# FAKEBOB-adversarial-attack/FAKEBOB

Hardware: AMD Instinct MI355X
Metric: NES iterations/sec (and scored-utts/sec) at samples_per_draw=50, 3 s@16 kHz (higher is better)
Workload: dtype f32 (GMM: two-term f16 split on MFMA, f32 accumulate, f32-equivalent; f32 MFCC; f64 NES)

## Files before the change

fakebob_amd/csrc/gmm_wide_kernel.hip:

```cpp
#include <float.h>
#include <cstdlib>
#include <type_traits>

#include "fb_kernels.h"
#include "gmm_split.h"

__device__ __forceinline__ void fb_glds16(const void *gsrc, unsigned lds_dst) {
  unsigned keep;
  asm volatile("s_mov_b32 %0, m0\n\ts_mov_b32 m0, %2\n\ts_nop 0\n\tglobal_load_lds_dwordx4 %1, off\n\ts_mov_b32 m0, %0"
               : "=&s"(keep) : "v"(gsrc), "s"(lds_dst) : "memory");
}
template <int N>
__device__ __forceinline__ void fb_glds16_run(const void *gsrc, unsigned lds_dst) {
  unsigned keep;
#define FB_GLDS_HEAD "s_mov_b32 %0, m0\n\ts_mov_b32 m0, %2\n\ts_nop 0\n\tglobal_load_lds_dwordx4 %1, off\n\t"
#define FB_GLDS_AT(o) "global_load_lds_dwordx4 %1, off offset:" #o "\n\t"
#define FB_GLDS_TAIL "s_mov_b32 m0, %0"
  if constexpr (N == 1)
    asm volatile(FB_GLDS_HEAD FB_GLDS_TAIL : "=&s"(keep) : "v"(gsrc), "s"(lds_dst) : "memory");
  else if constexpr (N == 2)
    asm volatile(FB_GLDS_HEAD FB_GLDS_AT(1024) FB_GLDS_TAIL : "=&s"(keep) : "v"(gsrc), "s"(lds_dst) : "memory");
  else if constexpr (N == 3)
    asm volatile(FB_GLDS_HEAD FB_GLDS_AT(1024) FB_GLDS_AT(2048) FB_GLDS_TAIL : "=&s"(keep) : "v"(gsrc), "s"(lds_dst) : "memory");
  else
    asm volatile(FB_GLDS_HEAD FB_GLDS_AT(1024) FB_GLDS_AT(2048) FB_GLDS_AT(3072) FB_GLDS_TAIL
                 : "=&s"(keep) : "v"(gsrc), "s"(lds_dst) : "memory");
#undef FB_GLDS_HEAD
#undef FB_GLDS_AT
#undef FB_GLDS_TAIL
}
template <int NITEMS, int NPIECE>
__device__ __forceinline__ void fb_fxw_fetch(const u32x4 *__restrict__ group_lane, unsigned lds_dst, int wv) {
  constexpr int TOT = NITEMS * NPIECE, PW = (TOT + 3) / 4;
  const u32x4 *src = group_lane + (size_t)wv * (PW * 64);
  const unsigned dst = lds_dst + (unsigned)wv * (PW * 1024);
// ... 10 lines not shown
__device__ __forceinline__ float fb_v_fma(float a, float b, float c) {
  float d;
  asm volatile("v_fma_f32 %0, %1, %2, %3" : "=v"(d) : "v"(a), "v"(b), "v"(c));
  return d;
}
__device__ __forceinline__ float fb_v_exp(float a) {
  float d;
  asm volatile("v_exp_f32 %0, %1" : "=v"(d) : "v"(a));
  return d;
}
__device__ __forceinline__ float fb_v_add(float a, float b) {
  float d;
  asm volatile("v_add_f32 %0, %1, %2" : "=v"(d) : "v"(a), "v"(b));
  return d;
}

#ifdef FB_FXW_COUNT
__device__ unsigned long long g_fxw_counts[4];
extern "C" int fb_debug_fxw_counts(unsigned long long *out) {
  if (hipMemcpyFromSymbol(out, HIP_SYMBOL(g_fxw_counts), sizeof(g_fxw_counts)) != hipSuccess) return -1;
  unsigned long long z[4] = {0, 0, 0, 0};
  return hipMemcpyToSymbol(HIP_SYMBOL(g_fxw_counts), z, sizeof(z)) == hipSuccess ? 0 : -1;
}
#define FXW_COUNT(i) do { if ((threadIdx.x & 63) == 0) atomicAdd(&g_fxw_counts[i], 1ull); } while (0)
#else
#define FXW_COUNT(i) do { } while (0)
#endif
#ifdef FB_FXW_STAMP
__device__ unsigned long long g_fxw_stamps[16];
extern "C" int fb_debug_fxw_stamps(unsigned long long *out) {
  return hipMemcpyFromSymbol(out, HIP_SYMBOL(g_fxw_stamps), sizeof(g_fxw_stamps)) == hipSuccess ? 0 : -1;
}
#define FXW_STAMP(i) do { if (blockIdx.x == 8 && threadIdx.x == 0) g_fxw_stamps[i] = wall_clock64(); } while (0)
#else
#define FXW_STAMP(i) do { } while (0)
#endif
#define FB_FXW_ROFF 64.0f
#define FB_FXW_SMAX 1.2676506002282294e30f
struct FbFxwUpd { float so0, so1, sn0, sn1; };

__device__ __forceinline__ void fb_fxw_slow_update(const f32x16 &p, float up, float rt, float mo, float so,
                                                   float *__restrict__ pm, float *__restrict__ ps, float &rn, bool need) {
  float tm = -3.0e38f;
#pragma unroll
  for (int r = 0; r < 16; ++r) tm = fmaxf(tm, __fmul_rn(p[r], up));
  const float mo_e = so > 0.0f ? mo : -INFINITY;
  const float mn = fmaxf(mo_e, __fadd_rn(rt, rintf(tm)));
  const float off = __fsub_rn(mn, rt);
  float a0 = __fmul_rn(so, __builtin_amdgcn_exp2f(__fsub_rn(mo_e, mn))), a1 = 0.0f;
#pragma unroll
  for (int r = 0; r < 16; r += 2) {
    a0 = __fadd_rn(a0, __builtin_amdgcn_exp2f(__fmaf_rn(p[r], up, -off)));
    a1 = __fadd_rn(a1, __builtin_amdgcn_exp2f(__fmaf_rn(p[r + 1], up, -off)));
  }
  if (need) {
    *pm = mn;
    *ps = __fadd_rn(a0, a1);
    rn = fmaxf(rn, mn);
  }
}

template <int NK, int NP, bool UPD, bool ZI = false, bool DEFERRED = false>
__device__ __forceinline__ void fb_fxw_step(const u32x4 *__restrict__ cur4, const u32x4 *__restrict__ nxt4, const bool pf0,
                                            int lane, u32x4 &z1, u32x4 &z2, const u32x4 (&b1)[2][NK],
                                            const u32x4 (&b2)[2][NK], const f32x16 &init0, const f32x16 &init1,
                                            f32x16 &out0, f32x16 &out1, const f32x16 &p0, const f32x16 &p1,
                                            float *__restrict__ ps, const float wd0, const float wd1, FbFxwUpd &u,
                                            const u32x4 *__restrict__ dsrc, unsigned ddst, const int dq0, const int dn) {
  constexpr int KP = 2 * NP, NG = KP * NK;
  constexpr int NS = 20;
  static_assert(NP >= 1 && NP <= 3 && NG >= 10, "slice layout");
  f32x16 x0, x1;
  if constexpr (ZI) {
#pragma unroll
    for (int r = 0; r < 16; ++r) { x0[r] = 0.0f; x1[r] = 0.0f; }
  } else {
    x0 = init0;
    x1 = init1;
  }
  constexpr int PD = NP == 1 ? 2 : 1;
  u32x4 s1[PD + 1], s2[PD + 1];
  float se0 = 0.f, se1 = 0.f, sd0 = 0.f, sd1 = 0.f;
  float ea0 = 0.f, ea1 = 0.f, eb0 = 0.f, eb1 = 0.f;
#pragma unroll
  for (int g = 0; g < NG; ++g) {
    const int c = g / KP, kk = g % KP;
    const int k = NP == 3 ? kk : (NP == 2 ? (kk < 2 ? kk : kk + 2) : kk + 4);
    if (kk == 0) {
#pragma unroll
      for (int cn = (c == 0 ? 1 : c + PD); cn <= c + PD && cn < NK; ++cn) {
        s1[cn % (PD + 1)] = cur4[(0 * NK + cn) * 64 + lane];
        if (NP >= 2) s2[cn % (PD + 1)] = cur4[(1 * NK + cn) * 64 + lane];
      }
    }
    const u32x4 &a1 = c == 0 ? z1 : s1[c % (PD + 1)], &a2 = c == 0 ? z2 : s2[c % (PD + 1)];
    if (k == 0) FB_FX_MFMA(a2, b1[0][c], x0);
    else if (k == 1) FB_FX_MFMA(a2, b1[1][c], x1);
    else if (k == 2) FB_FX_MFMA(a1, b2[0][c], x0);
    else if (k == 3) FB_FX_MFMA(a1, b2[1][c], x1);
    else if (k == 4) FB_FX_MFMA(a1, b1[0][c], x0);
    else FB_FX_MFMA(a1, b1[1][c], x1);
    if (pf0 && g == KP + 1) {
      z1 = nxt4[(0 * NK + 0) * 64 + lane];
      z2 = nxt4[(1 * NK + 0) * 64 + lane];
    }
    if (kk == (KP > 3 ? 3 : KP - 1) && c < dn) fb_glds16(dsrc + (dq0 + c) * 64, ddst + (unsigned)(dq0 + c) * 1024u);
    if constexpr (UPD) {
      const int m0 = (g * 4 * NS) / NG, m1 = ((g + 1) * 4 * NS) / NG;
#pragma unroll
      for (int mm = m0; mm < m1; ++mm) {
        const int sl = mm >> 2, part = mm & 3;
        const int r = sl - 1;
        const int ra = sl - 3;
        if (part == 0) {
          if (ra == 0) se0 = ea0;
          else if (ra == 1) sd0 = ea0;
          else if (ra >= 2 && ra <= 15 && !(ra & 1)) se0 = fb_v_add(se0, ea0);
          else if (ra >= 2 && ra <= 15) sd0 = fb_v_add(sd0, ea0);
        } else if (part == 1) {
          if (ra == 0) se1 = ea1;
          else if (ra == 1) sd1 = ea1;
          else if (ra >= 2 && ra <= 15 && !(ra & 1)) se1 = fb_v_add(se1, ea1);
          else if (ra >= 2 && ra <= 15) sd1 = fb_v_add(sd1, ea1);
          ea0 = eb0; ea1 = eb1;
        } else if (part == 2) {
          if (sl == 0) { u.so0 = ps[0]; u.so1 = ps[256]; }
          if (r >= 0 && r <= 15) eb0 = fb_v_exp(p0[r]);
        } else {
          if (r >= 0 && r <= 15) eb1 = fb_v_exp(p1[r]);
          if (sl == NS - 1) {
            u.sn0 = DEFERRED ? fb_v_fma(fb_v_add(se0, sd0), wd0, u.so0) : fb_v_add(fb_v_add(se0, sd0), u.so0);
            u.sn1 = DEFERRED ? fb_v_fma(fb_v_add(se1, sd1), wd1, u.so1) : fb_v_add(fb_v_add(se1, sd1), u.so1);
            ps[0] = u.sn0; ps[256] = u.sn1;
          }
        }
      }
    }
    __builtin_amdgcn_sched_barrier(0);
  }
  asm volatile("" : "+v"(x0), "+v"(x1));
  out0 = x0;
  out1 = x1;
}


typedef int i32x8 __attribute__((ext_vector_type(8)));
template <int NK, bool UPD>
__device__ __forceinline__ void fb_fxw_step6(const u32x4 *__restrict__ cur4, const u32x4 *__restrict__ nxt4, const bool pf0,
                                             int lane, u32x4 &z1, const u32x4 (&b1)[2][NK], const i32x8 (&fq)[2][3],
                                             const int (&fsc)[2][3], const f32x16 &init0, const f32x16 &init1,
                                             f32x16 &out0, f32x16 &out1, const f32x16 &p0, const f32x16 &p1,
                                             float *__restrict__ ps, FbFxwUpd &u, const u32x4 *__restrict__ dsrc, unsigned ddst,
                                             const int dq0, const int dn) {
  static_assert(NK == 5, "F6 item layout");
  constexpr int NM = 2 * NK, NG = NM + 8;
  constexpr int NS = 20, PD = 2;
  f32x16 x0 = init0, x1 = init1;
  u32x4 s1[PD + 1];
  i32x8 pa[4];
  int psc = 0, psh[4] = {0, 0, 0, 0};
  float se0 = 0.f, se1 = 0.f, sd0 = 0.f, sd1 = 0.f;
  float ea0 = 0.f, ea1 = 0.f, eb0 = 0.f, eb1 = 0.f;
  const unsigned char *ib = reinterpret_cast<const unsigned char *>(cur4);
#pragma unroll
  for (int g = 0; g < NG; ++g) {
    if (g < NM) {
      const int c = g / 2, kk = g % 2;
      if (kk == 0) {
#pragma unroll
        for (int cn = (c == 0 ? 1 : c + PD); cn <= c + PD && cn < NK; ++cn) s1[cn % (PD + 1)] = cur4[cn * 64 + lane];
        if (c == 0) {
          const u32x4 lo = *reinterpret_cast<const u32x4 *>(ib + 5120 + lane * 16);
          const uint2 hi = *reinterpret_cast<const uint2 *>(ib + 6144 + lane * 8);
          pa[0] = i32x8{(int)lo[0], (int)lo[1], (int)lo[2], (int)lo[3], (int)hi.x, (int)hi.y, 0, 0};
          psc = *reinterpret_cast<const int *>(ib + 9984 + lane * 4);
        } else if (c == 1) {
          const u32x4 lo = *reinterpret_cast<const u32x4 *>(ib + 8192 + lane * 16);
          pa[1] = i32x8{(int)lo[0], (int)lo[1], (int)lo[2], (int)lo[3], 0, 0, 0, 0};
        } else if (c == 2) {
          const u32x4 lo = *reinterpret_cast<const u32x4 *>(ib + 6656 + lane * 16);
          const uint2 hi = *reinterpret_cast<const uint2 *>(ib + 7680 + lane * 8);
          pa[2] = i32x8{(int)lo[0], (int)lo[1], (int)lo[2], (int)lo[3], (int)hi.x, (int)hi.y, 0, 0};
        } else if (c == 3) {
          const u32x4 lo = *reinterpret_cast<const u32x4 *>(ib + 9216 + (lane & 31) * 16);
          const uint2 hi = *reinterpret_cast<const uint2 *>(ib + 9728 + (lane & 31) * 8);
          pa[3] = i32x8{(int)lo[0], (int)lo[1], (int)lo[2], (int)lo[3], (int)hi.x, (int)hi.y, 0, 0};
        } else {
          psh[0] = psc; psh[1] = psc >> 16; psh[2] = psc >> 8; psh[3] = psc >> 24;
        }
      }
      const u32x4 &a1 = c == 0 ? z1 : s1[c % (PD + 1)];
      if (kk == 0) FB_FX_MFMA(a1, b1[0][c], x0);
      else FB_FX_MFMA(a1, b1[1][c], x1);
      if (pf0 && g == 3) z1 = nxt4[lane];
      if (kk == 1 && c < dn) fb_glds16(dsrc + (dq0 + c) * 64, ddst + (unsigned)(dq0 + c) * 1024u);
    } else {
      const int blk = (g - NM) / 2, hf = (g - NM) % 2;
      const int fb = blk == 0 || blk == 1 ? 0 : blk - 1;
      const int sa = psh[blk];
      if (blk == 1) {
        if (hf == 0) x0 = __builtin_amdgcn_mfma_scale_f32_32x32x64_f8f6f4(pa[1], fq[0][fb], x0, 4, 2, 0, sa, 0, fsc[0][fb]);
        else x1 = __builtin_amdgcn_mfma_scale_f32_32x32x64_f8f6f4(pa[1], fq[1][fb], x1, 4, 2, 0, sa, 0, fsc[1][fb]);
      } else {
        if (hf == 0) x0 = __builtin_amdgcn_mfma_scale_f32_32x32x64_f8f6f4(pa[blk], fq[0][fb], x0, 2, 2, 0, sa, 0, fsc[0][fb]);
        else x1 = __builtin_amdgcn_mfma_scale_f32_32x32x64_f8f6f4(pa[blk], fq[1][fb], x1, 2, 2, 0, sa, 0, fsc[1][fb]);
      }
    }
    if constexpr (UPD) {
      const int m0 = (g * 4 * NS) / NG, m1 = ((g + 1) * 4 * NS) / NG;
#pragma unroll
      for (int mm = m0; mm < m1; ++mm) {
        const int sl = mm >> 2, part = mm & 3;
        const int r = sl - 1, ra = sl - 3;
        if (part == 0) {
          if (ra == 0) se0 = ea0;
          else if (ra == 1) sd0 = ea0;
          else if (ra >= 2 && ra <= 15 && !(ra & 1)) se0 = fb_v_add(se0, ea0);
          else if (ra >= 2 && ra <= 15) sd0 = fb_v_add(sd0, ea0);
        } else if (part == 1) {
          if (ra == 0) se1 = ea1;
          else if (ra == 1) sd1 = ea1;
          else if (ra >= 2 && ra <= 15 && !(ra & 1)) se1 = fb_v_add(se1, ea1);
          else if (ra >= 2 && ra <= 15) sd1 = fb_v_add(sd1, ea1);
          ea0 = eb0; ea1 = eb1;
        } else if (part == 2) {
          if (sl == 0) { u.so0 = ps[0]; u.so1 = ps[256]; }
          if (r >= 0 && r <= 15) eb0 = fb_v_exp(p0[r]);
        } else {
          if (r >= 0 && r <= 15) eb1 = fb_v_exp(p1[r]);
          if (sl == NS - 1) {
            u.sn0 = fb_v_add(fb_v_add(se0, sd0), u.so0);
            u.sn1 = fb_v_add(fb_v_add(se1, sd1), u.so1);
            ps[0] = u.sn0; ps[256] = u.sn1;
          }
        }
      }
    }
    __builtin_amdgcn_sched_barrier(0);
  }
  asm volatile("" : "+v"(x0), "+v"(x1));
  out0 = x0;
  out1 = x1;
}

template <int NK, int M>
__global__ __launch_bounds__(256, 1) void k_gmm_fx2w(FbGmmDev g, const float *__restrict__ feats,
                                                     const int *__restrict__ n_rows_ptr, int n_chunks,
                                                     int rows_cap, float *__restrict__ part_m,
                                                     float *__restrict__ part_s, int xcd_map) {
  if (g.stop && *g.stop) return;
  extern __shared__ __attribute__((aligned(16))) float lds[];
  constexpr int IMG4 = 2 * NK * 64;
  constexpr int NI = M + 1;
  constexpr int GA = (NI + 1) / 2, GB = NI - GA;
  FXW_STAMP(0);
  const int n_rows = *n_rows_ptr;
  int strip_i, gchunk;
  if (xcd_map) {
    const int lin = blockIdx.x, per = 8 / xcd_map;
    const int xcd = lin & 7, idx = lin >> 3;
    gchunk = xcd / per;
    strip_i = idx * per + (xcd % per);
  } else {
    strip_i = blockIdx.x;
    gchunk = blockIdx.y;
  }
  const int n_sub = g.fxw_sub > 1 ? g.fxw_sub : 1, grid_chunks = n_chunks / n_sub;
  const int strip0 = strip_i * 256;
  if (strip0 >= n_rows) return;
  const int tid = threadIdx.x, lane = tid & 63, w = tid >> 6;
  const int h = lane >> 5, j = lane & 31;
  constexpr int PAD4 = 192;
  constexpr int SLOTB4 = GA * IMG4 + PAD4;
  const u32x4 *slot0 = reinterpret_cast<const u32x4 *>(lds);
  float *st_m = lds + (NI * IMG4 + 2 * PAD4) * 4;
  float *st_s = st_m + M * 512;
// ... 236 lines not shown
  const int wv = __builtin_amdgcn_readfirstlane(w);
  const unsigned ring_lds = (unsigned)(unsigned long long)(__attribute__((address_space(3))) void *)lds;
  auto item4 = [&](int jj) { return jj < GA ? jj * IMG4 : SLOTB4 + (jj - GA) * IMG4; };
  const unsigned guard = slow ? 0u : __float_as_uint(FB_FXW_SMAX) + 1u;
  auto settle = [&](const f32x16 &p0, const f32x16 &p1, float *pm, float *ps, const float (&rt)[2], const FbFxwUpd &u) {
    const unsigned worst = max(__float_as_uint(u.sn0), __float_as_uint(u.sn1));
    FXW_COUNT(0);
#ifdef FB_FXW_COUNT
    {
      const float th0 = __builtin_amdgcn_logf(u.so0) - 25.0f, th1 = __builtin_amdgcn_logf(u.so1) - 25.0f;
      int n = 0;
#pragma unroll
      for (int r = 0; r < 16; ++r)
        if (__builtin_amdgcn_ballot_w64(!(p0[r] < th0) || !(p1[r] < th1)) == 0ull) ++n;
      if ((threadIdx.x & 63) == 0) atomicAdd(&g_fxw_counts[3], (unsigned long long)n);
    }
#endif
    if (__builtin_expect(__builtin_amdgcn_ballot_w64(worst >= guard) != 0ull, 0)) {
      FXW_COUNT(1);
      fb_fxw_slow_update(p0, up[0], rt[0], pm[0], u.so0, pm, ps, rn[0], __float_as_uint(u.sn0) >= guard);
      fb_fxw_slow_update(p1, up[1], rt[1], pm[256], u.so1, pm + 256, ps + 256, rn[1], __float_as_uint(u.sn1) >= guard);
    }
  };
  auto update = [&](const f32x16 &v0, const f32x16 &v1, int model) {
    float *pm = st_m + (2 * model) * 256 + tid, *ps = st_s + (2 * model) * 256 + tid;
    fb_fxw_slow_update(v0, up[0], rc[0], pm[0], ps[0], pm, ps, rn[0], true);
    fb_fxw_slow_update(v1, up[1], rc[1], pm[256], ps[256], pm + 256, ps + 256, rn[1], true);
  };
  auto publish = [&]() {
    asm volatile("s_waitcnt vmcnt(0)" ::: "memory");
    __syncthreads();
  };

  f32x16 hq[2], acc[2][2], zero;
#pragma unroll
  for (int r = 0; r < 16; ++r) {
    hq[0][r] = 0.f; hq[1][r] = 0.f; zero[r] = 0.f;
    acc[0][0][r] = -1.0e30f; acc[0][1][r] = -1.0e30f; acc[1][0][r] = -1.0e30f; acc[1][1][r] = -1.0e30f;
  }
  FbFxwUpd uu;
  float wd[2] = {1.0f, 1.0f};
  FXW_STAMP(3);
  fb_fxw_fetch<GA, NPIECE>(gimg + (size_t)tile_of(0) * NI * IMG4 + lane, ring_lds, wv);
  publish();
  FXW_STAMP(4);
  u32x4 z1, z2;
  constexpr int PW_A = (GA * NPIECE + 3) / 4, PW_B = (GB * NPIECE + 3) / 4;
  auto tile = [&](auto pc, const int t) __attribute__((always_inline)) {
    constexpr int P = decltype(pc)::value;
    rp[0] = rc[0]; rp[1] = rc[1];
    if (__builtin_expect(__builtin_amdgcn_ballot_w64(rn[0] > rc[0] || rn[1] > rc[1] || wd[0] != 1.0f || wd[1] != 1.0f) != 0ull, 0)) {
      FXW_COUNT(2);
#pragma unroll
      for (int hf = 0; hf < 2; ++hf) {
        rn[hf] = fminf(fmaxf(rn[hf], __shfl_xor(rn[hf], 32, 64)), 4.0e6f);
        rc[hf] = slow ? 0.0f : rn[hf];
        set_ref(hf, rc[hf]);
        wd[hf] = __builtin_amdgcn_exp2f(rp[hf] - rc[hf]);
        if (!slow) {
#pragma unroll
          for (int m = 0; m < M; ++m) {
            float *pm = st_m + (2 * m + hf) * 256 + tid, *ps = st_s + (2 * m + hf) * 256 + tid;
            *ps = *ps * __builtin_amdgcn_exp2f(*pm - rc[hf]);
            *pm = rc[hf];
          }
        }
      }
    }
    const u32x4 *srcB = gimg + ((size_t)tile_of(t) * NI + GA) * IMG4 + (size_t)wv * (PW_B * 64) + lane;
    const u32x4 *srcA = gimg + (size_t)tile_of(t + 1) * NI * IMG4 + (size_t)wv * (PW_A * 64) + lane;
    const unsigned dstB = ring_lds + SLOTB4 * 16 + (unsigned)wv * (PW_B * 1024), dstA = ring_lds + (unsigned)wv * (PW_A * 1024);
#pragma clang loop unroll(full)
    for (int jj = 0; jj < NI; ++jj) {
      const bool first_of_group = (jj == 0 || jj == GA);
      const u32x4 *cur4 = slot0 + item4(jj);
      if (first_of_group) {
        z1 = cur4[(0 * NK + 0) * 64 + lane];
        z2 = cur4[(1 * NK + 0) * 64 + lane];
      }
      const int gs = jj < GA ? jj : jj - GA;
      const int pw = jj < GA ? PW_B : PW_A, dq0 = 5 * gs;
      int dn = dq0 < pw ? (pw - dq0 < 5 ? pw - dq0 : 5) : 0;
      const u32x4 *dsrc = jj < GA ? srcB : srcA;
      const unsigned ddst = jj < GA ? dstB : dstA;
      if (first_of_group) {
#pragma unroll
        for (int q = 0; q < dn; ++q) fb_glds16(dsrc + q * 64, ddst + (unsigned)q * 1024u);
        dn = 0;
      }
      const bool pf0 = (jj + 1 < NI && jj + 1 != GA);
      const u32x4 *nxt4 = slot0 + item4(jj + 1 < NI ? jj + 1 : 0);
      constexpr bool DEFER = M >= 3;
      if (jj == 0) {
        if constexpr (DEFER) {
          float *pm = st_m + (2 * (M - 2)) * 256 + tid, *ps = st_s + (2 * (M - 2)) * 256 + tid;
          fb_fxw_step<NK, 3, true, true, true>(cur4, nxt4, pf0, lane, z1, z2, bq1, bq2, zero, zero, hq[0], hq[1], acc[(M - 2) & 1][0], acc[(M - 2) & 1][1], ps, wd[0], wd[1], uu, dsrc, ddst, dq0, dn);
          settle(acc[(M - 2) & 1][0], acc[(M - 2) & 1][1], pm, ps, rp, uu);
        } else {
          fb_fxw_step<NK, 3, false, true>(cur4, nxt4, pf0, lane, z1, z2, bq1, bq2, zero, zero, hq[0], hq[1], zero, zero, st_s, 1.f, 1.f, uu, dsrc, ddst, dq0, dn);
        }
      } else if (jj == 1) {
        float *pm = st_m + (2 * (M - 1)) * 256 + tid, *ps = st_s + (2 * (M - 1)) * 256 + tid;
        fb_fxw_step<NK, 3, true, false, true>(cur4, nxt4, pf0, lane, z1, z2, bx1, bx2, hq[0], hq[1], hq[0], hq[1], acc[(M - 1) & 1][0], acc[(M - 1) & 1][1], ps, wd[0], wd[1], uu, dsrc, ddst, dq0, dn);
        settle(acc[(M - 1) & 1][0], acc[(M - 1) & 1][1], pm, ps, rp, uu);
      } else if (jj == 2) {
        float *pm = st_m + tid, *ps = st_s + tid;
        if constexpr (P == 6)
          fb_fxw_step6<NK, true>(cur4, nxt4, pf0, lane, z1, bx1, fq, fsc, hq[0], hq[1], acc[1][0], acc[1][1], hq[0], hq[1], ps, uu, dsrc, ddst, dq0, dn);
        else
          fb_fxw_step<NK, P, true>(cur4, nxt4, pf0, lane, z1, z2, bx1, bx2, hq[0], hq[1], acc[1][0], acc[1][1], hq[0], hq[1], ps, 1.f, 1.f, uu,
                                   dsrc, ddst, dq0, dn);
        settle(hq[0], hq[1], pm, ps, rc, uu);
      } else if (DEFER && jj == NI - 1) {
        if constexpr (P == 6)
          fb_fxw_step6<NK, false>(cur4, nxt4, pf0, lane, z1, bx1, fq, fsc, hq[0], hq[1], acc[(jj - 1) & 1][0], acc[(jj - 1) & 1][1],
                                  zero, zero, st_s, uu, dsrc, ddst, dq0, dn);
        else
          fb_fxw_step<NK, P, false>(cur4, nxt4, pf0, lane, z1, z2, bx1, bx2, hq[0], hq[1], acc[(jj - 1) & 1][0], acc[(jj - 1) & 1][1],
                                    zero, zero, st_s, 1.f, 1.f, uu, dsrc, ddst, dq0, dn);
      } else {
        float *pm = st_m + (2 * (jj - 2)) * 256 + tid, *ps = st_s + (2 * (jj - 2)) * 256 + tid;
        if constexpr (P == 6)
          fb_fxw_step6<NK, true>(cur4, nxt4, pf0, lane, z1, bx1, fq, fsc, hq[0], hq[1], acc[(jj - 1) & 1][0], acc[(jj - 1) & 1][1],
                                 acc[(jj - 2) & 1][0], acc[(jj - 2) & 1][1], ps, uu, dsrc, ddst, dq0, dn);
        else
          fb_fxw_step<NK, P, true>(cur4, nxt4, pf0, lane, z1, z2, bx1, bx2, hq[0], hq[1], acc[(jj - 1) & 1][0], acc[(jj - 1) & 1][1],
                                   acc[(jj - 2) & 1][0], acc[(jj - 2) & 1][1], ps, 1.f, 1.f, uu, dsrc, ddst, dq0, dn);
        settle(acc[(jj - 2) & 1][0], acc[(jj - 2) & 1][1], pm, ps, rc, uu);
      }
      if (jj == GA - 1 || jj == NI - 1) publish();
    }
  };
  {
    int t = 0;
    for (; t < n_p3; ++t) tile(std::integral_constant<int, 3>{}, t);
    for (; t < n_p36; ++t) tile(std::integral_constant<int, 6>{}, t);
    for (; t < n_p32; ++t) tile(std::integral_constant<int, 2>{}, t);
    for (; t < n_t; ++t) tile(std::integral_constant<int, 1>{}, t);
  }
  FXW_STAMP(5);
  asm volatile("s_waitcnt vmcnt(0)" ::: "memory");
  auto tail_update = [&](const f32x16 &v0, const f32x16 &v1, int model) {
    if (slow) { update(v0, v1, model); return; }
    float *pm = st_m + (2 * model) * 256 + tid, *ps = st_s + (2 * model) * 256 + tid;
    FbFxwUpd u;
    u.so0 = ps[0]; u.so1 = ps[256];
    float e0 = __builtin_amdgcn_exp2f(v0[0]), d0 = __builtin_amdgcn_exp2f(v0[1]);
    float e1 = __builtin_amdgcn_exp2f(v1[0]), d1 = __builtin_amdgcn_exp2f(v1[1]);
#pragma unroll
    for (int r = 2; r < 16; r += 2) {
      e0 = __fadd_rn(e0, __builtin_amdgcn_exp2f(v0[r])); d0 = __fadd_rn(d0, __builtin_amdgcn_exp2f(v0[r + 1]));
      e1 = __fadd_rn(e1, __builtin_amdgcn_exp2f(v1[r])); d1 = __fadd_rn(d1, __builtin_amdgcn_exp2f(v1[r + 1]));
    }
    u.sn0 = __fadd_rn(__fadd_rn(e0, d0), u.so0);
    u.sn1 = __fadd_rn(__fadd_rn(e1, d1), u.so1);
    ps[0] = u.sn0; ps[256] = u.sn1;
    settle(v0, v1, pm, ps, rc, u);
  };
  if constexpr (M >= 3) tail_update(acc[(M - 2) & 1][0], acc[(M - 2) & 1][1], M - 2);
  tail_update(acc[(M - 1) & 1][0], acc[(M - 1) & 1][1], M - 1);
  FXW_STAMP(6);

#pragma unroll
  for (int m = 0; m < M; ++m)
#pragma unroll
    for (int hf = 0; hf < 2; ++hf) {
      const float ms = st_m[(2 * m + hf) * 256 + tid], s0 = st_s[(2 * m + hf) * 256 + tid];
      const float ln2f = 0.693147182464599609375f;
      const float mm = __fmul_rn(ms, ln2f);
      const float dd = __fmaf_rn(ms, -1.9046542999e-9f, __fmaf_rn(ms, ln2f, -mm));
      const float ss = __fmaf_rn(s0, __fmaf_rn(__fmul_rn(0.5f, dd), dd, dd), s0);
      const float m2 = __shfl_xor(mm, 32, 64), s2 = __shfl_xor(ss, 32, 64);
      const float mx = fmaxf(mm, m2);
      const float sx = ss * __expf(mm - mx) + s2 * __expf(m2 - mx);
      if (h == 0 && rows[hf] < n_rows) {
        const int mg = m == 0 ? 0 : g.pass_first + m - 1;
        const size_t o = ((size_t)chunk_i * g.M + mg) * rows_cap + rows[hf];
        part_m[o] = mx;
        part_s[o] = sx;
      }
    }
  }
  FXW_STAMP(7);
}


template <int NK, bool PICK>
__global__ __launch_bounds__(256, 1) void k_gsel_w(FbGmmDev g, const float *__restrict__ feats, const int *__restrict__ n_rows_ptr,
                                                   int tiles_per_chunk, int n_chunks, float *__restrict__ gmax,
                                                   const float *__restrict__ tau, float *__restrict__ gval,
                                                   unsigned char *__restrict__ gid, int *__restrict__ gcnt, int xcd_map,
                                                   int tiles_a) {
  if (g.stop && *g.stop) return;
// ... 35 lines not shown
    fb_fx_frame_load<NK>(g, feats, rows[hf], n_rows, h, ft[hf]);
  }
#pragma unroll
  for (int hf = 0; hf < 2; ++hf) {
    (void)fb_fx_frame_make<NK, true>(g, feats, ft[hf], rows[hf], n_rows, h, bx1[hf], bx2[hf], bq1[hf], bq2[hf]);
#pragma unroll
    for (int c = 0; c < NK; ++c) asm volatile("" : "+a"(bx2[hf][c]), "+a"(bq1[hf][c]), "+a"(bq2[hf][c]));
    __builtin_amdgcn_sched_barrier(0);
  }
  FXW_STAMP(9);
  float tauv[2] = {FLT_MAX, FLT_MAX};
  float4 *gb[2] = {nullptr, nullptr};
  if constexpr (PICK) {
#pragma unroll
    for (int hf = 0; hf < 2; ++hf) {
      if (rows[hf] < n_rows) tauv[hf] = tau[rows[hf]];
      gb[hf] = reinterpret_cast<float4 *>(gval) + ((size_t)(rows[hf] < n_rows ? rows[hf] : 0) * n_chunks + chunk_i) * capc * 4;
    }
    s_cnt[tid] = 0;
  }
  const int tile0 = chunk_i * tiles_per_chunk;
  const int n_tiles_run = PICK ? tiles_per_chunk : tiles_a;
  const int n_grp = n_tiles_run / TS;
  const u32x4 *gimg = g.images_fx + (size_t)tile0 * 2 * IMG4;
  const int wv = __builtin_amdgcn_readfirstlane(w);
  const unsigned ring_lds = (unsigned)(unsigned long long)(__attribute__((address_space(3))) void *)lds;
  auto publish = [&]() {
    asm volatile("s_waitcnt vmcnt(0)" ::: "memory");
    __syncthreads();
  };
  f32x16 hq[2][2], zero;
#pragma unroll
  for (int r = 0; r < 16; ++r) { hq[0][0][r] = 0.f; hq[0][1][r] = 0.f; hq[1][0][r] = 0.f; hq[1][1][r] = 0.f; zero[r] = 0.f; }
  FbFxwUpd uu;
  FXW_STAMP(10);
  fb_fxw_fetch<NIG, NPIECE>(gimg + lane, ring_lds, wv);
  publish();
  FXW_STAMP(11);
  u32x4 z1, z2;
  auto epilogue = [&](const int tl, const int par) {
#pragma unroll
    for (int hf = 0; hf < 2; ++hf) {
      const f32x16 &v = hq[par][hf];
      float m = fmaxf(fmaxf(v[0], v[1]), v[2]);
#pragma unroll
      for (int r = 3; r < 15; r += 2) m = fmaxf(fmaxf(m, v[r]), v[r + 1]);
      m = fmaxf(m, v[15]);
      if constexpr (!PICK) {
        s_mx[((w * 16 + (tl & 15)) * 2 + hf) * 64 + lane] = m;
      } else {
        if (m >= tauv[hf]) {
          const int rl = w * 64 + hf * 32 + j;
          const int k = atomicAdd(&s_cnt[rl], 1);
          float4 *dst = gb[hf] + (size_t)k * 4;
          dst[0] = make_float4(v[0], v[1], v[2], v[3]);
          dst[1] = make_float4(v[4], v[5], v[6], v[7]);
          dst[2] = make_float4(v[8], v[9], v[10], v[11]);
          dst[3] = make_float4(v[12], v[13], v[14], v[15]);
          s_gid[rl * capc + k] = (unsigned char)(2 * tl + h);
        }
      }
    }
    if constexpr (!PICK) {
      if ((tl & 15) == 15 || tl == tiles_a - 1) {
        const int nt = (tl & 15) + 1, per_row = 2 * nt, NGr = 2 * n_chunks * tiles_a, pos0 = 2 * (chunk_i * tiles_a + (tl & ~15));
        __builtin_amdgcn_fence(__ATOMIC_RELEASE, "wavefront");
        __builtin_amdgcn_wave_barrier();
// ... 7 lines not shown
        __builtin_amdgcn_wave_barrier();
        __builtin_amdgcn_fence(__ATOMIC_ACQUIRE, "wavefront");
      }
    }
  };
  for (int gp = 0; gp < n_grp; gp += 2) {
    const u32x4 *srcB = gimg + (size_t)min(gp + 1, n_grp - 1) * SLOT4 + (size_t)wv * (PW * 64) + lane;
    const u32x4 *srcA = gimg + (size_t)min(gp + 2, n_grp - 1) * SLOT4 + (size_t)wv * (PW * 64) + lane;
    const unsigned dstB = ring_lds + SLOT4 * 16 + (unsigned)wv * (PW * 1024), dstA = ring_lds + (unsigned)wv * (PW * 1024);
#pragma clang loop unroll(full)
    for (int jj = 0; jj < 2 * NIG; ++jj) {
      const bool in_b = jj >= NIG;
      const int gs = jj % NIG;
      const u32x4 *cur4 = slot0 + (in_b ? SLOT4 : 0) + gs * IMG4;
      const u32x4 *nxt4 = slot0 + (in_b ? SLOT4 : 0) + (gs + 1 < NIG ? gs + 1 : 0) * IMG4;
      const bool pf0 = gs + 1 < NIG;
      if (gs == 0) {
        z1 = cur4[(0 * NK + 0) * 64 + lane];
        z2 = cur4[(1 * NK + 0) * 64 + lane];
      }
      const u32x4 *dsrc = in_b ? srcA : srcB;
      const unsigned ddst = in_b ? dstA : dstB;
      const int dq0 = 5 * gs;
      int dn = dq0 < PW ? (PW - dq0 < 5 ? PW - dq0 : 5) : 0;
      if (gs == 0) {
#pragma unroll
        for (int q = 0; q < dn; ++q) fb_glds16(dsrc + q * 64, ddst + (unsigned)q * 1024u);
        dn = 0;
      }
      constexpr int dummy = 0; (void)dummy;
      const int par = (jj >> 1) & 1;
      const int tl = gp * TS + (jj >> 1);
      if (!(jj & 1)) {
        fb_fxw_step<NK, 3, false, true>(cur4, nxt4, pf0, lane, z1, z2, bq1, bq2, zero, zero, hq[par][0], hq[par][1], zero, zero, lds, 1.f, 1.f,
                                        uu, dsrc, ddst, dq0, dn);
        if (tl > 0) epilogue(tl - 1, par ^ 1);
      } else {
        fb_fxw_step<NK, 3, false, false>(cur4, nxt4, pf0, lane, z1, z2, bx1, bx2, hq[par][0], hq[par][1], hq[par][0], hq[par][1], zero, zero, lds,
                                         1.f, 1.f, uu, dsrc, ddst, dq0, dn);
      }
      if (gs == NIG - 1) publish();
    }
  }
  epilogue(n_tiles_run - 1, 1);
  FXW_STAMP(12);
  if constexpr (PICK) {
    __syncthreads();
    for (int i = tid; i < 256 * (capc / 4); i += 256) {
      const int r2 = i / (capc / 4), q = i - r2 * (capc / 4);
      const int rg = strip0 + r2;
      if (rg < n_rows)
        reinterpret_cast<unsigned *>(gid + ((size_t)rg * n_chunks + chunk_i) * capc)[q] = reinterpret_cast<const unsigned *>(s_gid + r2 * capc)[q];
    }
    if (strip0 + tid < n_rows) gcnt[(size_t)(strip0 + tid) * n_chunks + chunk_i] = s_cnt[tid];
  }
  FXW_STAMP(13);
}

bool fb_gsel_w_applies(const FbGmmDev &g, int n_chunks) {
  const bool off = getenv("FB_GSEL_NARROW") != nullptr;
  if (off || g.NKF != 5 || (g.C & 31) != 0 || (g.D & 3) != 0 || g.n_tiles % n_chunks != 0) return false;
  const int tpc = g.n_tiles / n_chunks;
  return (tpc & 3) == 0 && tpc <= 128;
}
int fb_gsel_w_tiles_a(const FbGmmDev &g, int n_chunks, int nsel) {
  const int tpc = g.n_tiles / n_chunks;
  const bool full = getenv("FB_GSEL_A_HALF") == nullptr;
  if (!full && (tpc & 7) == 0 && n_chunks * tpc >= 3 * nsel) return tpc / 2;
  return tpc;
}
void fb_launch_gsel_w(hipStream_t s, const FbGmmDev &g, const float *feats, const int *n_rows_ptr, int rows_cap, int n_chunks, int pick,
                      float *gmax, const float *tau, float *gval, unsigned char *gid, int *gcnt, int tiles_a) {
// ... 78 lines not shown
```

Before: 12460.

## Spread per-model logsumexp updates evenly across fused MFMA steps of the wide GMM kernel

Before, each MFMA step in the wide GMM kernel carried the whole exp/accumulate update for exactly one earlier model's score tile. Now the update work of all models is spread evenly over the remaining steps, so a single step can finish one model's slices and start the next model's. Running state moves into a per-model FbFxwRun struct, and a third accumulator buffer is added to hold the extra model in flight. The aim is to balance the VALU work hidden behind each step's MFMAs and remove stalls from uneven step lengths, at the cost of more live registers. Cycle-stamp probes are also added, but only behind a debug macro.

New measurement: 12630, median of 6. No clear change (+1.4%).

```diff
diff --git a/fakebob_amd/csrc/gmm_wide_kernel.hip b/fakebob_amd/csrc/gmm_wide_kernel.hip
--- a/fakebob_amd/csrc/gmm_wide_kernel.hip
+++ b/fakebob_amd/csrc/gmm_wide_kernel.hip
@@ -1,6 +1,7 @@
 #include <float.h>
 #include <cstdlib>
 #include <type_traits>
+#include <utility>
 
 #include "fb_kernels.h"
 #include "gmm_split.h"
@@ -77,6 +78,16 @@
   return hipMemcpyFromSymbol(out, HIP_SYMBOL(g_fxw_stamps), sizeof(g_fxw_stamps)) == hipSuccess ? 0 : -1;
 }
 #define FXW_STAMP(i) do { if (blockIdx.x == 8 && threadIdx.x == 0) g_fxw_stamps[i] = wall_clock64(); } while (0)
+__device__ unsigned long long g_fxw_steps[64];
+extern "C" int fb_debug_fxw_steps(unsigned long long *out) {
+  return hipMemcpyFromSymbol(out, HIP_SYMBOL(g_fxw_steps), sizeof(g_fxw_steps)) == hipSuccess ? 0 : -1;
+}
+#define FXW_CLOCK(v)                                                                      \
+  do {                                                                                    \
+    __builtin_amdgcn_sched_barrier(0);                                                    \
+    asm volatile("s_memtime %0\n\ts_waitcnt lgkmcnt(0)" : "=s"(v) :: "memory");          \
+    __builtin_amdgcn_sched_barrier(0);                                                    \
+  } while (0)
 #else
 #define FXW_STAMP(i) do { } while (0)
 #endif
@@ -105,15 +116,62 @@
   }
 }
 
-template <int NK, int NP, bool UPD, bool ZI = false, bool DEFERRED = false>
+struct FbFxwRun { float se0, se1, sd0, sd1, ea0, ea1, eb0, eb1; FbFxwUpd u; };
+
+template <bool DEFERRED>
+__device__ __forceinline__ void fb_fxw_part(const int mm, FbFxwRun &q, const f32x16 &p0, const f32x16 &p1, float *__restrict__ ps,
+                                            const float wd0, const float wd1) {
+  constexpr int NS = 20;
+  const int sl = mm >> 2, part = mm & 3;
+  const int r = sl - 1;
+  const int ra = sl - 3;
+  if (part == 0) {
+    if (ra == 0) q.se0 = q.ea0;
+    else if (ra == 1) q.sd0 = q.ea0;
+    else if (ra >= 2 && ra <= 15 && !(ra & 1)) q.se0 = fb_v_add(q.se0, q.ea0);
+    else if (ra >= 2 && ra <= 15) q.sd0 = fb_v_add(q.sd0, q.ea0);
+  } else if (part == 1) {
+    if (ra == 0) q.se1 = q.ea1;
+    else if (ra == 1) q.sd1 = q.ea1;
+    else if (ra >= 2 && ra <= 15 && !(ra & 1)) q.se1 = fb_v_add(q.se1, q.ea1);
+    else if (ra >= 2 && ra <= 15) q.sd1 = fb_v_add(q.sd1, q.ea1);
+    q.ea0 = q.eb0; q.ea1 = q.eb1;
+  } else if (part == 2) {
+    if (sl == 0) { q.u.so0 = ps[0]; q.u.so1 = ps[256]; }
+    if (r >= 0 && r <= 15) q.eb0 = fb_v_exp(p0[r]);
+  } else {
+    if (r >= 0 && r <= 15) q.eb1 = fb_v_exp(p1[r]);
+    if (sl == NS - 1) {
+      q.u.sn0 = DEFERRED ? fb_v_fma(fb_v_add(q.se0, q.sd0), wd0, q.u.so0) : fb_v_add(fb_v_add(q.se0, q.sd0), q.u.so0);
+      q.u.sn1 = DEFERRED ? fb_v_fma(fb_v_add(q.se1, q.sd1), wd1, q.u.so1) : fb_v_add(fb_v_add(q.se1, q.sd1), q.u.so1);
+      ps[0] = q.u.sn0; ps[256] = q.u.sn1;
+    }
+  }
+}
+
+template <int NG, int A0, int B0, int A1, int B1, bool DEFERRED>
+__device__ __forceinline__ void fb_fxw_gap(const int g, FbFxwRun &qa, const f32x16 &va0, const f32x16 &va1, float *__restrict__ psa,
+                                           FbFxwRun &qb, const f32x16 &vb0, const f32x16 &vb1, float *__restrict__ psb,
+                                           const float wd0, const float wd1) {
+  constexpr int N0 = 4 * (B0 - A0), NT = N0 + 4 * (B1 - A1);
+  const int m0 = (g * NT) / NG, m1 = ((g + 1) * NT) / NG;
+#pragma unroll
+  for (int mm = m0; mm < m1; ++mm) {
+    if (mm < N0) fb_fxw_part<DEFERRED>(4 * A0 + mm, qa, va0, va1, psa, wd0, wd1);
+    else fb_fxw_part<false>(4 * A1 + mm - N0, qb, vb0, vb1, psb, 1.0f, 1.0f);
+  }
+}
+
+template <int NK, int NP, bool ZI = false, int A0 = 0, int B0 = 0, int A1 = 0, int B1 = 0, bool DEFERRED = false>
 __device__ __forceinline__ void fb_fxw_step(const u32x4 *__restrict__ cur4, const u32x4 *__restrict__ nxt4, const bool pf0,
                                             int lane, u32x4 &z1, u32x4 &z2, const u32x4 (&b1)[2][NK],
                                             const u32x4 (&b2)[2][NK], const f32x16 &init0, const f32x16 &init1,
-                                            f32x16 &out0, f32x16 &out1, const f32x16 &p0, const f32x16 &p1,
-                                            float *__restrict__ ps, const float wd0, const float wd1, FbFxwUpd &u,
+                                            f32x16 &out0, f32x16 &out1,
+                                            FbFxwRun &qa, const f32x16 &va0, const f32x16 &va1, float *__restrict__ psa,
+                                            FbFxwRun &qb, const f32x16 &vb0, const f32x16 &vb1, float *__restrict__ psb,
+                                            const float wd0, const float wd1,
                                             const u32x4 *__restrict__ dsrc, unsigned ddst, const int dq0, const int dn) {
   constexpr int KP = 2 * NP, NG = KP * NK;
-  constexpr int NS = 20;
   static_assert(NP >= 1 && NP <= 3 && NG >= 10, "slice layout");
   f32x16 x0, x1;
   if constexpr (ZI) {
@@ -125,8 +183,6 @@
   }
   constexpr int PD = NP == 1 ? 2 : 1;
   u32x4 s1[PD + 1], s2[PD + 1];
-  float se0 = 0.f, se1 = 0.f, sd0 = 0.f, sd1 = 0.f;
-  float ea0 = 0.f, ea1 = 0.f, eb0 = 0.f, eb1 = 0.f;
 #pragma unroll
   for (int g = 0; g < NG; ++g) {
     const int c = g / KP, kk = g % KP;
@@ -150,37 +206,7 @@
       z2 = nxt4[(1 * NK + 0) * 64 + lane];
     }
     if (kk == (KP > 3 ? 3 : KP - 1) && c < dn) fb_glds16(dsrc + (dq0 + c) * 64, ddst + (unsigned)(dq0 + c) * 1024u);
-    if constexpr (UPD) {
-      const int m0 = (g * 4 * NS) / NG, m1 = ((g + 1) * 4 * NS) / NG;
-#pragma unroll
-      for (int mm = m0; mm < m1; ++mm) {
-        const int sl = mm >> 2, part = mm & 3;
-        const int r = sl - 1;
-        const int ra = sl - 3;
-        if (part == 0) {
-          if (ra == 0) se0 = ea0;
-          else if (ra == 1) sd0 = ea0;
-          else if (ra >= 2 && ra <= 15 && !(ra & 1)) se0 = fb_v_add(se0, ea0);
-          else if (ra >= 2 && ra <= 15) sd0 = fb_v_add(sd0, ea0);
-        } else if (part == 1) {
-          if (ra == 0) se1 = ea1;
-          else if (ra == 1) sd1 = ea1;
-          else if (ra >= 2 && ra <= 15 && !(ra & 1)) se1 = fb_v_add(se1, ea1);
-          else if (ra >= 2 && ra <= 15) sd1 = fb_v_add(sd1, ea1);
-          ea0 = eb0; ea1 = eb1;
-        } else if (part == 2) {
-          if (sl == 0) { u.so0 = ps[0]; u.so1 = ps[256]; }
-          if (r >= 0 && r <= 15) eb0 = fb_v_exp(p0[r]);
-        } else {
-          if (r >= 0 && r <= 15) eb1 = fb_v_exp(p1[r]);
-          if (sl == NS - 1) {
-            u.sn0 = DEFERRED ? fb_v_fma(fb_v_add(se0, sd0), wd0, u.so0) : fb_v_add(fb_v_add(se0, sd0), u.so0);
-            u.sn1 = DEFERRED ? fb_v_fma(fb_v_add(se1, sd1), wd1, u.so1) : fb_v_add(fb_v_add(se1, sd1), u.so1);
-            ps[0] = u.sn0; ps[256] = u.sn1;
-          }
-        }
-      }
-    }
+    fb_fxw_gap<NG, A0, B0, A1, B1, DEFERRED>(g, qa, va0, va1, psa, qb, vb0, vb1, psb, wd0, wd1);
     __builtin_amdgcn_sched_barrier(0);
   }
   asm volatile("" : "+v"(x0), "+v"(x1));
@@ -190,22 +216,21 @@
 
 
 typedef int i32x8 __attribute__((ext_vector_type(8)));
-template <int NK, bool UPD>
+template <int NK, int A0, int B0, int A1, int B1>
 __device__ __forceinline__ void fb_fxw_step6(const u32x4 *__restrict__ cur4, const u32x4 *__restrict__ nxt4, const bool pf0,
                                              int lane, u32x4 &z1, const u32x4 (&b1)[2][NK], const i32x8 (&fq)[2][3],
                                              const int (&fsc)[2][3], const f32x16 &init0, const f32x16 &init1,
-                                             f32x16 &out0, f32x16 &out1, const f32x16 &p0, const f32x16 &p1,
-                                             float *__restrict__ ps, FbFxwUpd &u, const u32x4 *__restrict__ dsrc, unsigned ddst,
-                                             const int dq0, const int dn) {
+                                             f32x16 &out0, f32x16 &out1,
+                                             FbFxwRun &qa, const f32x16 &va0, const f32x16 &va1, float *__restrict__ psa,
+                                             FbFxwRun &qb, const f32x16 &vb0, const f32x16 &vb1, float *__restrict__ psb,
+                                             const u32x4 *__restrict__ dsrc, unsigned ddst, const int dq0, const int dn) {
   static_assert(NK == 5, "F6 item layout");
   constexpr int NM = 2 * NK, NG = NM + 8;
-  constexpr int NS = 20, PD = 2;
+  constexpr int PD = 2;
   f32x16 x0 = init0, x1 = init1;
   u32x4 s1[PD + 1];
   i32x8 pa[4];
   int psc = 0, psh[4] = {0, 0, 0, 0};
-  float se0 = 0.f, se1 = 0.f, sd0 = 0.f, sd1 = 0.f;
-  float ea0 = 0.f, ea1 = 0.f, eb0 = 0.f, eb1 = 0.f;
   const unsigned char *ib = reinterpret_cast<const unsigned char *>(cur4);
 #pragma unroll
   for (int g = 0; g < NG; ++g) {
@@ -251,42 +276,24 @@
         else x1 = __builtin_amdgcn_mfma_scale_f32_32x32x64_f8f6f4(pa[blk], fq[1][fb], x1, 2, 2, 0, sa, 0, fsc[1][fb]);
       }
     }
-    if constexpr (UPD) {
-      const int m0 = (g * 4 * NS) / NG, m1 = ((g + 1) * 4 * NS) / NG;
-#pragma unroll
-      for (int mm = m0; mm < m1; ++mm) {
-        const int sl = mm >> 2, part = mm & 3;
-        const int r = sl - 1, ra = sl - 3;
-        if (part == 0) {
-          if (ra == 0) se0 = ea0;
-          else if (ra == 1) sd0 = ea0;
-          else if (ra >= 2 && ra <= 15 && !(ra & 1)) se0 = fb_v_add(se0, ea0);
-          else if (ra >= 2 && ra <= 15) sd0 = fb_v_add(sd0, ea0);
-        } else if (part == 1) {
-          if (ra == 0) se1 = ea1;
-          else if (ra == 1) sd1 = ea1;
-          else if (ra >= 2 && ra <= 15 && !(ra & 1)) se1 = fb_v_add(se1, ea1);
-          else if (ra >= 2 && ra <= 15) sd1 = fb_v_add(sd1, ea1);
-          ea0 = eb0; ea1 = eb1;
-        } else if (part == 2) {
-          if (sl == 0) { u.so0 = ps[0]; u.so1 = ps[256]; }
-          if (r >= 0 && r <= 15) eb0 = fb_v_exp(p0[r]);
-        } else {
-          if (r >= 0 && r <= 15) eb1 = fb_v_exp(p1[r]);
-          if (sl == NS - 1) {
-            u.sn0 = fb_v_add(fb_v_add(se0, sd0), u.so0);
-            u.sn1 = fb_v_add(fb_v_add(se1, sd1), u.so1);
-            ps[0] = u.sn0; ps[256] = u.sn1;
-          }
-        }
-      }
-    }
+    fb_fxw_gap<NG, A0, B0, A1, B1, false>(g, qa, va0, va1, psa, qb, vb0, vb1, psb, 1.0f, 1.0f);
     __builtin_amdgcn_sched_barrier(0);
   }
   asm volatile("" : "+v"(x0), "+v"(x1));
   out0 = x0;
   out1 = x1;
 }
+
+template <class F, int... J>
+__device__ __forceinline__ void fb_fxw_static_for_(F &&f, std::integer_sequence<int, J...>) {
+  (f(std::integral_constant<int, J>{}), ...);
+}
+template <int N, class F>
+__device__ __forceinline__ void fb_fxw_static_for(F &&f) {
+  fb_fxw_static_for_(f, std::make_integer_sequence<int, N>{});
+}
+constexpr int fb_fxw_nu(int M) { return M >= 3 ? M - 2 : 1; }
+constexpr int fb_fxw_pos(int M, int i) { return 20 * fb_fxw_nu(M) * i / (M - 1); }
 
 template <int NK, int M>
 __global__ __launch_bounds__(256, 1) void k_gmm_fx2w(FbGmmDev g, const float *__restrict__ feats,
@@ -589,18 +596,24 @@
     __syncthreads();
   };
 
-  f32x16 hq[2], acc[2][2], zero;
+  f32x16 hq[2], acc[3][2], zero;
 #pragma unroll
   for (int r = 0; r < 16; ++r) {
     hq[0][r] = 0.f; hq[1][r] = 0.f; zero[r] = 0.f;
-    acc[0][0][r] = -1.0e30f; acc[0][1][r] = -1.0e30f; acc[1][0][r] = -1.0e30f; acc[1][1][r] = -1.0e30f;
-  }
-  FbFxwUpd uu;
+#pragma unroll
+    for (int a = 0; a < 3; ++a) { acc[a][0][r] = -1.0e30f; acc[a][1][r] = -1.0e30f; }
+  }
+  auto vals = [&](const int m) -> f32x16 (&)[2] { return m == 0 ? hq : acc[(m - 1) % 3]; };
+  FbFxwRun run[2] = {}, qd = {};
   float wd[2] = {1.0f, 1.0f};
   FXW_STAMP(3);
   fb_fxw_fetch<GA, NPIECE>(gimg + (size_t)tile_of(0) * NI * IMG4 + lane, ring_lds, wv);
   publish();
   FXW_STAMP(4);
+#ifdef FB_FXW_STAMP
+  unsigned long long clk0;
+  FXW_CLOCK(clk0);
+#endif
   u32x4 z1, z2;
   constexpr int PW_A = (GA * NPIECE + 3) / 4, PW_B = (GB * NPIECE + 3) / 4;
   auto tile = [&](auto pc, const int t) __attribute__((always_inline)) {
@@ -624,12 +637,21 @@
         }
       }
     }
+#ifdef FB_FXW_STAMP
+    const int cls = P == 3 ? 0 : (P == 6 ? 1 : (P == 2 ? 2 : 3));
+    const int c_lo = P == 3 ? 0 : (P == 6 ? n_p3 : (P == 2 ? n_p36 : n_p32)), c_hi = P == 3 ? n_p3 : (P == 6 ? n_p36 : (P == 2 ? n_p32 : n_t));
+    const bool stamp_tile = blockIdx.x == 8 && tid == 0 && t == (c_lo + 1 < c_hi ? c_lo + 1 : c_lo);
+    unsigned long long tst[NI + 1];
+#endif
     const u32x4 *srcB = gimg + ((size_t)tile_of(t) * NI + GA) * IMG4 + (size_t)wv * (PW_B * 64) + lane;
     const u32x4 *srcA = gimg + (size_t)tile_of(t + 1) * NI * IMG4 + (size_t)wv * (PW_A * 64) + lane;
     const unsigned dstB = ring_lds + SLOTB4 * 16 + (unsigned)wv * (PW_B * 1024), dstA = ring_lds + (unsigned)wv * (PW_A * 1024);
-#pragma clang loop unroll(full)
-    for (int jj = 0; jj < NI; ++jj) {
-      const bool first_of_group = (jj == 0 || jj == GA);
+    fb_fxw_static_for<NI>([&](auto jc) __attribute__((always_inline)) {
+      constexpr int jj = decltype(jc)::value;
+#ifdef FB_FXW_STAMP
+      FXW_CLOCK(tst[jj]);
+#endif
+      constexpr bool first_of_group = (jj == 0 || jj == GA);
       const u32x4 *cur4 = slot0 + item4(jj);
       if (first_of_group) {
         z1 = cur4[(0 * NK + 0) * 64 + lane];
@@ -647,46 +669,49 @@
       }
       const bool pf0 = (jj + 1 < NI && jj + 1 != GA);
       const u32x4 *nxt4 = slot0 + item4(jj + 1 < NI ? jj + 1 : 0);
+      float *const ps_of = st_s + tid;
       constexpr bool DEFER = M >= 3;
-      if (jj == 0) {
+      if constexpr (jj == 0) {
         if constexpr (DEFER) {
-          float *pm = st_m + (2 * (M - 2)) * 256 + tid, *ps = st_s + (2 * (M - 2)) * 256 + tid;
-          fb_fxw_step<NK, 3, true, true, true>(cur4, nxt4, pf0, lane, z1, z2, bq1, bq2, zero, zero, hq[0], hq[1], acc[(M - 2) & 1][0], acc[(M - 2) & 1][1], ps, wd[0], wd[1], uu, dsrc, ddst, dq0, dn);
-          settle(acc[(M - 2) & 1][0], acc[(M - 2) & 1][1], pm, ps, rp, uu);
+          constexpr int md = M - 2;
+          fb_fxw_step<NK, 3, true, 0, 20, 0, 0, true>(cur4, nxt4, pf0, lane, z1, z2, bq1, bq2, zero, zero, hq[0], hq[1],
+                                                       qd, vals(md)[0], vals(md)[1], ps_of + 2 * md * 256, qd, zero, zero, st_s,
+                                                       wd[0], wd[1], dsrc, ddst, dq0, dn);
+          settle(vals(md)[0], vals(md)[1], st_m + 2 * md * 256 + tid, ps_of + 2 * md * 256, rp, qd.u);
         } else {
-          fb_fxw_step<NK, 3, false, true>(cur4, nxt4, pf0, lane, z1, z2, bq1, bq2, zero, zero, hq[0], hq[1], zero, zero, st_s, 1.f, 1.f, uu, dsrc, ddst, dq0, dn);
+          fb_fxw_step<NK, 3, true>(cur4, nxt4, pf0, lane, z1, z2, bq1, bq2, zero, zero, hq[0], hq[1], qd, zero, zero, st_s, qd,
+                                   zero, zero, st_s, 1.f, 1.f, dsrc, ddst, dq0, dn);
         }
-      } else if (jj == 1) {
-        float *pm = st_m + (2 * (M - 1)) * 256 + tid, *ps = st_s + (2 * (M - 1)) * 256 + tid;
-        fb_fxw_step<NK, 3, true, false, true>(cur4, nxt4, pf0, lane, z1, z2, bx1, bx2, hq[0], hq[1], hq[0], hq[1], acc[(M - 1) & 1][0], acc[(M - 1) & 1][1], ps, wd[0], wd[1], uu, dsrc, ddst, dq0, dn);
-        settle(acc[(M - 1) & 1][0], acc[(M - 1) & 1][1], pm, ps, rp, uu);
-      } else if (jj == 2) {
-        float *pm = st_m + tid, *ps = st_s + tid;
+      } else if constexpr (jj == 1) {
+        constexpr int md = M - 1;
+        fb_fxw_step<NK, 3, false, 0, 20, 0, 0, true>(cur4, nxt4, pf0, lane, z1, z2, bx1, bx2, hq[0], hq[1], hq[0], hq[1],
+                                                      qd, vals(md)[0], vals(md)[1], ps_of + 2 * md * 256, qd, zero, zero, st_s,
+                                                      wd[0], wd[1], dsrc, ddst, dq0, dn);
+        settle(vals(md)[0], vals(md)[1], st_m + 2 * md * 256 + tid, ps_of + 2 * md * 256, rp, qd.u);
+      } else {
+        constexpr int lo = fb_fxw_pos(M, jj - 2), hi = fb_fxw_pos(M, jj - 1);
+        constexpr int ma = lo / 20, mb = ma + 1;
+        constexpr int A0 = lo - 20 * ma, B0 = hi - 20 * ma < 20 ? hi - 20 * ma : 20, B1 = hi > 20 * mb ? hi - 20 * mb : 0;
+        f32x16 (&dst)[2] = vals(jj - 1);
         if constexpr (P == 6)
-          fb_fxw_step6<NK, true>(cur4, nxt4, pf0, lane, z1, bx1, fq, fsc, hq[0], hq[1], acc[1][0], acc[1][1], hq[0], hq[1], ps, uu, dsrc, ddst, dq0, dn);
+          fb_fxw_step6<NK, A0, B0, 0, B1>(cur4, nxt4, pf0, lane, z1, bx1, fq, fsc, hq[0], hq[1], dst[0], dst[1],
+                                          run[ma & 1], vals(ma)[0], vals(ma)[1], ps_of + 2 * ma * 256,
+                                          run[mb & 1], vals(mb)[0], vals(mb)[1], ps_of + 2 * mb * 256, dsrc, ddst, dq0, dn);
         else
-          fb_fxw_step<NK, P, true>(cur4, nxt4, pf0, lane, z1, z2, bx1, bx2, hq[0], hq[1], acc[1][0], acc[1][1], hq[0], hq[1], ps, 1.f, 1.f, uu,
-                                   dsrc, ddst, dq0, dn);
-        settle(hq[0], hq[1], pm, ps, rc, uu);
-      } else if (DEFER && jj == NI - 1) {
-        if constexpr (P == 6)
-          fb_fxw_step6<NK, false>(cur4, nxt4, pf0, lane, z1, bx1, fq, fsc, hq[0], hq[1], acc[(jj - 1) & 1][0], acc[(jj - 1) & 1][1],
-                                  zero, zero, st_s, uu, dsrc, ddst, dq0, dn);
-        else
-          fb_fxw_step<NK, P, false>(cur4, nxt4, pf0, lane, z1, z2, bx1, bx2, hq[0], hq[1], acc[(jj - 1) & 1][0], acc[(jj - 1) & 1][1],
-                                    zero, zero, st_s, 1.f, 1.f, uu, dsrc, ddst, dq0, dn);
-      } else {
-        float *pm = st_m + (2 * (jj - 2)) * 256 + tid, *ps = st_s + (2 * (jj - 2)) * 256 + tid;
-        if constexpr (P == 6)
-          fb_fxw_step6<NK, true>(cur4, nxt4, pf0, lane, z1, bx1, fq, fsc, hq[0], hq[1], acc[(jj - 1) & 1][0], acc[(jj - 1) & 1][1],
-                                 acc[(jj - 2) & 1][0], acc[(jj - 2) & 1][1], ps, uu, dsrc, ddst, dq0, dn);
-        else
-          fb_fxw_step<NK, P, true>(cur4, nxt4, pf0, lane, z1, z2, bx1, bx2, hq[0], hq[1], acc[(jj - 1) & 1][0], acc[(jj - 1) & 1][1],
-                                   acc[(jj - 2) & 1][0], acc[(jj - 2) & 1][1], ps, 1.f, 1.f, uu, dsrc, ddst, dq0, dn);
-        settle(acc[(jj - 2) & 1][0], acc[(jj - 2) & 1][1], pm, ps, rc, uu);
+          fb_fxw_step<NK, P, false, A0, B0, 0, B1>(cur4, nxt4, pf0, lane, z1, z2, bx1, bx2, hq[0], hq[1], dst[0], dst[1],
+                                                   run[ma & 1], vals(ma)[0], vals(ma)[1], ps_of + 2 * ma * 256,
+                                                   run[mb & 1], vals(mb)[0], vals(mb)[1], ps_of + 2 * mb * 256, 1.f, 1.f,
+                                                   dsrc, ddst, dq0, dn);
+        if constexpr (B0 == 20) settle(vals(ma)[0], vals(ma)[1], st_m + 2 * ma * 256 + tid, ps_of + 2 * ma * 256, rc, run[ma & 1].u);
+        if constexpr (B1 == 20) settle(vals(mb)[0], vals(mb)[1], st_m + 2 * mb * 256 + tid, ps_of + 2 * mb * 256, rc, run[mb & 1].u);
       }
       if (jj == GA - 1 || jj == NI - 1) publish();
-    }
+    });
+#ifdef FB_FXW_STAMP
+    FXW_CLOCK(tst[NI]);
+    if (stamp_tile)
+      for (int k = 0; k <= NI; ++k) g_fxw_steps[cls * 12 + k] = tst[k];
+#endif
   };
   {
     int t = 0;
@@ -695,6 +720,11 @@
     for (; t < n_p32; ++t) tile(std::integral_constant<int, 2>{}, t);
     for (; t < n_t; ++t) tile(std::integral_constant<int, 1>{}, t);
   }
+#ifdef FB_FXW_STAMP
+  unsigned long long clk1;
+  FXW_CLOCK(clk1);
+  if (blockIdx.x == 8 && tid == 0) { g_fxw_steps[48] = clk0; g_fxw_steps[49] = clk1; }
+#endif
   FXW_STAMP(5);
   asm volatile("s_waitcnt vmcnt(0)" ::: "memory");
   auto tail_update = [&](const f32x16 &v0, const f32x16 &v1, int model) {
@@ -714,8 +744,8 @@
     ps[0] = u.sn0; ps[256] = u.sn1;
     settle(v0, v1, pm, ps, rc, u);
   };
-  if constexpr (M >= 3) tail_update(acc[(M - 2) & 1][0], acc[(M - 2) & 1][1], M - 2);
-  tail_update(acc[(M - 1) & 1][0], acc[(M - 1) & 1][1], M - 1);
+  if constexpr (M >= 3) tail_update(vals(M - 2)[0], vals(M - 2)[1], M - 2);
+  tail_update(vals(M - 1)[0], vals(M - 1)[1], M - 1);
   FXW_STAMP(6);
 
 #pragma unroll
@@ -817,7 +847,7 @@
   f32x16 hq[2][2], zero;
 #pragma unroll
   for (int r = 0; r < 16; ++r) { hq[0][0][r] = 0.f; hq[0][1][r] = 0.f; hq[1][0][r] = 0.f; hq[1][1][r] = 0.f; zero[r] = 0.f; }
-  FbFxwUpd uu;
+  FbFxwRun uu = {};
   FXW_STAMP(10);
   fb_fxw_fetch<NIG, NPIECE>(gimg + lane, ring_lds, wv);
   publish();
@@ -891,12 +921,12 @@
       const int par = (jj >> 1) & 1;
       const int tl = gp * TS + (jj >> 1);
       if (!(jj & 1)) {
-        fb_fxw_step<NK, 3, false, true>(cur4, nxt4, pf0, lane, z1, z2, bq1, bq2, zero, zero, hq[par][0], hq[par][1], zero, zero, lds, 1.f, 1.f,
-                                        uu, dsrc, ddst, dq0, dn);
+        fb_fxw_step<NK, 3, true>(cur4, nxt4, pf0, lane, z1, z2, bq1, bq2, zero, zero, hq[par][0], hq[par][1], uu, zero, zero, lds,
+                                 uu, zero, zero, lds, 1.f, 1.f, dsrc, ddst, dq0, dn);
         if (tl > 0) epilogue(tl - 1, par ^ 1);
       } else {
-        fb_fxw_step<NK, 3, false, false>(cur4, nxt4, pf0, lane, z1, z2, bx1, bx2, hq[par][0], hq[par][1], hq[par][0], hq[par][1], zero, zero, lds,
-                                         1.f, 1.f, uu, dsrc, ddst, dq0, dn);
+        fb_fxw_step<NK, 3, false>(cur4, nxt4, pf0, lane, z1, z2, bx1, bx2, hq[par][0], hq[par][1], hq[par][0], hq[par][1], uu, zero, zero, lds,
+                                  uu, zero, zero, lds, 1.f, 1.f, dsrc, ddst, dq0, dn);
       }
       if (gs == NIG - 1) publish();
     }
```
